# peterWon/D-LIOM

Hardware: AMD Instinct MI355X
Metric: scans/sec (64-beam x 1024 pts -> 10 cm 3D submap) (higher is better)
Workload: dtype f32 transforms + u16 voxels/u64 sums (rtcsm), f64 (ceres); 1 GPU; config2 W-dense: 64x1024 scan, all returns matched (adaptive voxel filters neutralised), RTCSM3D + CeresScanMatcher3D(hi+lo) + insertion(hi+lo); N_hi=65536, N_lo=65536, C=35937, linear_window=1, angular_window=5, rescored_candidates_last=2, box_kernel_variant=0, map_scans=20, grids_inserted_into=2, parallelism=replicas x1

## Files before the change

### d-liom_amd/csrc/internal.h

```cpp
#ifndef DLIOM_CSRC_INTERNAL_H_
#define DLIOM_CSRC_INTERNAL_H_

#include <hip/hip_runtime.h>

#include <chrono>
#include <cstddef>
#include <cstdint>
#include <memory>
#include <string>
#include <vector>

#include "../../include/dliom.h"
#include "pinned_layout.h"

namespace dliom {

void set_last_error(const char* what, hipError_t e, const char* file, int line);

#define DLIOM_HIP_TRY(expr)                                          \
  do {                                                               \
    hipError_t _e = (expr);                                          \
    if (_e != hipSuccess) {                                          \
      ::dliom::set_last_error(#expr, _e, __FILE__, __LINE__);        \
      return DLIOM_ERR_HIP;                                          \
// ... 35 lines not shown
  const uint16_t* dense;
  int dense_stride;
  int dense_bricks;
  int dense_off[3];
};

struct MemoryLedger {
  int64_t grids = 0, leaf_table_bytes = 0, leaf_pool_bytes = 0, mirror_bytes = 0;
  int64_t mirror_budget = 0;
  int64_t outlier_table_bytes = 0;
  int64_t probability_grid_bytes = 0;
  int64_t points_xray_bytes = 0;
  int64_t mirrors_refused = 0;
};

}

struct dliom_ctx {
  std::shared_ptr<dliom::MemoryLedger> ledger = std::make_shared<dliom::MemoryLedger>();
  int device = 0;
  hipStream_t stream = nullptr;
  bool owns_stream = false;
  dliom::DevBuf points;
  dliom::DevBuf cand;
  dliom::DevBuf sums;
  dliom::DevBuf bounds;
  dliom::DevBuf rescore;
  dliom::DevBuf partials;
  dliom::DevBuf misc;
  dliom::DevBuf sort_tmp;
  dliom::DevBuf voxel;
  dliom::DevBuf box_tables;
  dliom::DevBuf box_counters;
  dliom::DevBuf box_extents;
  dliom::DevBuf csm_arrivals;
  dliom::DevBuf box_error;
  dliom::DevBuf deskew_flags;
  unsigned deskew_flag_total = 0;
  unsigned deskew_launch_id = 0;
  int64_t deskew_records_checked = 0, deskew_overflows = 0, deskew_fixed_hits = 0;
  int64_t assemble_recorded = 0, assemble_recomputed = 0, assemble_fixed = 0, assemble_overflows = 0;
  dliom::DevBuf zero_words;
  bool zero_words_ready = false;
  bool box_error_zeroed = false;
  bool force_dense_score = false;
  int tuning[DLIOM_TUNE_COUNT] = {3, 4096, 0};
  bool last_score_used_box = false;
  int last_score_mapping = -1;
  int last_box_refusal = 0;
  int last_box_variant = -1;
  void* pinned = nullptr;
  unsigned* done_word = nullptr;
  unsigned done_seq = 0;
  int64_t voxel_unpacked_reruns = 0;
  int64_t read_backs = 0;
  int64_t poll_fallbacks = 0;
  int64_t host_syncs = 0;
  dliom::DevBuf batch;
  dliom::DevBuf xray_leaves, xray_cells;
  dliom::DevBuf surf, surf_out;
  dliom::DevBuf painter;
  int64_t painter_launches = 0, painter_pairs = 0, painter_texels_uploaded = 0;
  dliom::DevBuf compress, compress_out;
  bool surf_tables_ready = false;
  dliom::DevBuf outlier;
  void* batch_pinned = nullptr;
  size_t batch_pinned_bytes = 0;
  int reserve_batch_pinned(size_t bytes);
  int num_cus = 256;
  unsigned func_attr_set = 0;
  hipStream_t aux_stream = nullptr;
  hipEvent_t aux_fork = nullptr;
  dliom::DevBuf aux_scratch;
  void* aux_pinned = nullptr;
  int aux_histogram_size = 0;
  unsigned aux_seq = 0;
  bool aux_enqueued = false;
  const dliom_cloud* aux_cloud = nullptr;
  float aux_rotation[4] = {1.f, 0.f, 0.f, 0.f};
  bool aux_has_rotation = false;
  bool hist_expect_big = true;
  int hist_poll_us = 150;
  std::chrono::steady_clock::time_point hist_enqueued_at;
  hipStream_t hist_big_stream = nullptr;
  hipEvent_t hist_fork = nullptr, hist_join = nullptr;
  bool profiling = false;
  unsigned profiling_mask = ~0u;
  struct Span {
    hipEvent_t a, b;
    int id;
  };
  std::vector<Span> spans;
  std::vector<hipEvent_t> event_pool;
  double kernel_ms[DLIOM_KERNEL_COUNT] = {};
  int64_t kernel_launches[DLIOM_KERNEL_COUNT] = {};
  dliom_rtcsm_stats last_rtcsm = {};
  void* rtcsm_state = nullptr;
  void (*rtcsm_state_free)(void*) = nullptr;

  int begin_span(int id);
  void end_span(int span);
  int collect_spans();
};

struct dliom_grid {
  dliom_ctx* ctx = nullptr;
  float resolution = 0.f;
  int bits = 1;
  uint32_t* d_table = nullptr;
  uint16_t* d_pool = nullptr;
  int32_t* d_slot_coord = nullptr;
  uint32_t* d_count = nullptr;
  int64_t capacity = 0;
  int64_t used_upper = 1;
  unsigned* h_count_slot = nullptr;
  unsigned insert_seq = 0, applied_seq = 0;
  int64_t upper_at_insert = 0;
  uint16_t* d_dense = nullptr;
  int dense_stride = 0;
  int dense_bricks = 0;
  int dense_off[3] = {0, 0, 0};
  bool dense_windowed = false;
  int64_t dense_rebuilds = 0;
  int ensure_dense();
  int ensure_dense_for(const int centre[3], int radius_cells);
  void drop_dense();
  dliom::GridView view() const;
  std::shared_ptr<dliom::MemoryLedger> ledger;
  int64_t booked_table = 0, booked_pool = 0, booked_mirror = 0;
  int64_t mirror_bytes() const { return d_dense != nullptr ? static_cast<int64_t>(dense_bricks) * dense_bricks * dense_bricks * 128 : 0; }
  void book();
  int ensure_bits(int needed_bits);
  int ensure_capacity(int64_t additional_slots);
  int shrink_to_fit();
  int refresh_count(int64_t* count);
};

struct dliom_cloud {
  dliom_ctx* ctx = nullptr;
  int64_t n = 0;
  int64_t n_padded = 0;
  float* d_x = nullptr;
  float* d_y = nullptr;
  float* d_z = nullptr;
  float* d_xs = nullptr;
  float* d_ys = nullptr;
  float* d_zs = nullptr;
  float max_norm = 0.f;
  float abs_max[3] = {-1.f, -1.f, -1.f};
  bool owned_by_ctx_scratch = false;
  void* base = nullptr;
  size_t base_bytes = 0;
  int device = 0;
  bool morton_ready = false;
  unsigned* d_chunk_order = nullptr;
  unsigned* d_chunk_order_big = nullptr;
};

struct dliom_inserter {
  dliom_ctx* ctx = nullptr;
  int num_free_space_voxels = 0;
  std::vector<uint16_t> hit_table, miss_table;
  uint16_t* d_tables = nullptr;
};


// ... 27 lines not shown
constexpr float kPadCoordinate = 1.0e7f;
int stage_cloud(dliom_ctx* ctx, const float* points_xyz, int64_t n, dliom_cloud* out,
                size_t scratch_offset_bytes = 0);
float cloud_max_norm(const float* points_xyz, int64_t n);
size_t staged_cloud_bytes(int64_t n);
int alloc_device_cloud(dliom_ctx* ctx, int64_t n, dliom_cloud** out, float** x, float** y, float** z);
int finish_device_cloud(dliom_ctx* ctx, dliom_cloud* cloud, float max_norm);
int finish_device_cloud_from(dliom_ctx* ctx, dliom_cloud* cloud, float max_norm, const float* sx, const float* sy, const float* sz);
int ensure_morton(dliom_ctx* ctx, const dliom_cloud* cloud);
struct Soa {
  const float *x, *y, *z, *w;
  int64_t n;
};
int voxel_filter_arrays(dliom_ctx* ctx, const Soa& in, float size, float* ox, float* oy, float* oz, float* ow,
                        int64_t* n_out);
int voxel_filter_arrays_enqueue(dliom_ctx* ctx, const Soa& in, float size, float* ox, float* oy, float* oz, float* ow,
                                const unsigned** d_total, const unsigned** d_unpackable);
int compact_equal_arrays(dliom_ctx* ctx, const Soa& in, const unsigned char* kinds, unsigned char want, float* ox,
                         float* oy, float* oz, int64_t* n_out,
                         const void* also_src = nullptr, unsigned also_words = 0, void* also_dst = nullptr);
int compact_equal_arrays_enqueue(dliom_ctx* ctx, const Soa& in, const unsigned char* kinds, unsigned char want, float* ox,
                                 float* oy, float* oz, const unsigned* n_dev, const unsigned** d_total);
int needed_bits_for_cell_range(int min_index, int max_index);
int project_to_image_on_device(const dliom_grid* grid, const double transform7[7], const uint8_t** image, int32_t* width,
                               int32_t* height, double* ox, double* oy, double* resolution);
int surf_features_on_device(dliom_ctx* ctx, const uint8_t* image, int width, int height, const dliom_surf_options& options,
                            const float** keypoints, const float** descriptors, int* count);
int xray_texture_on_device(const dliom_grid* grid, const double global_submap_pose7[7], const uint8_t** cells, int32_t* width,
                           int32_t* height, double* resolution, double slice_pose7[7]);
int surf_check_options(const dliom_surf_options* options);

constexpr size_t align256(size_t bytes) { return (bytes + 255) & ~static_cast<size_t>(255); }
constexpr unsigned blocks_of(int64_t n, int threads) { return static_cast<unsigned>((n + threads - 1) / threads); }
struct FillJob {
  void* p;
  size_t bytes;
  unsigned value;
};
int fill_multi(dliom_ctx* ctx, const FillJob* jobs, int num_jobs, hipStream_t stream = nullptr);
struct GatherJob {
  const void* src;
  unsigned words;
  unsigned stride = 1;
};
int gather_to_pinned(dliom_ctx* ctx, const GatherJob* jobs, int num_jobs, void* pinned_dst, hipStream_t stream = nullptr,
                     unsigned* done_word = nullptr, unsigned done_seq = 0);
int wait_done(dliom_ctx* ctx, hipStream_t stream, const unsigned* done_word, unsigned done_seq, int max_poll_us = 150);
unsigned next_done_seq(dliom_ctx* ctx);
int gather_and_wait(dliom_ctx* ctx, const GatherJob* jobs, int num_jobs, void* pinned_dst);
int zero_words(dliom_ctx* ctx, unsigned** out);
int device_block_alloc(int device, size_t need, void** p, size_t* bytes);
void device_block_free(int device, void* p, size_t bytes);
struct CompactScratch {
  unsigned *keep, *inclusive, *max_sq;
  int* index;
  void* tmp;
  size_t tmp_bytes;
  void* extra;
};
int carve_compact(dliom_ctx* ctx, int64_t n, CompactScratch* s, size_t extra_bytes = 0, size_t zeroed_extra_bytes = 0);
int empty_cloud(dliom_ctx* ctx, dliom_cloud** out);
int max_of_kept(dliom_ctx* ctx, const float* x, const float* y, const float* z, int64_t n, const CompactScratch& s);
int scan_kept(dliom_ctx* ctx, int64_t n, const CompactScratch& s);
int read_kept(dliom_ctx* ctx, int64_t n, const CompactScratch& s, const GatherJob* more, int64_t* kept, float* max_sq,
              unsigned* more_host);
int emit_kept(dliom_ctx* ctx, const float* x, const float* y, const float* z, int64_t n, const CompactScratch& s, int64_t kept,
              float max_sq, dliom_cloud** out, int32_t* kept_index);
int compact_kept(dliom_ctx* ctx, const dliom_cloud* in, const CompactScratch& s, const unsigned* flag_word, unsigned* flag,
                 dliom_cloud** out, int32_t* kept_index, int64_t capacity, int64_t* num_kept);
int gather_batch_attributes(dliom_ctx* ctx, const int* d_index, int64_t kept, const float* src_intensities, const float* src_colors,
                            float* dst_intensities, float* dst_colors);
int compact_batch(dliom_points_batch* batch, const CompactScratch& s, const unsigned* flag_word, unsigned* flag, int64_t* num_kept);
struct DevicePoints {
  const float4* xyzt;
  const float* intensities;
};
int assemble_from_sensor_points(dliom_ctx* ctx, dliom_trajectory* traj, int64_t cloud_time, const float* points_xyzt, const DevicePoints* device_points,
                                int64_t n, const double sensor_to_tracking[7], dliom_cloud** out, float origin[3], int32_t* kept_index,
                                int64_t capacity, int64_t* num_kept, const float* intensities, AttrBlock* kept_intensities);
int timed_cloud_view(const dliom_timed_cloud* cloud, const dliom_ctx* ctx, int64_t* n, const float4** d_xyzt, const float** d_intensities,
                     float* front_t);
int timed_cloud_origin_index(const dliom_timed_cloud* cloud, bool* has, const float** d_origin_index);
int std_sort_order_enqueue(dliom_ctx* ctx, const float* d_keys, int n, const int** d_order, const int** d_status);
int launch_sequential_sums(dliom_ctx* ctx, int method, const GridView& gv, const dliom_cloud& cloud, const float4* d_rot,
                           int R, const float* d_trans, const unsigned* d_list, const unsigned* d_count, unsigned count,
                           DevBuf* scratch, float* d_ksums);
int sequential_sum_method(int64_t num_points);
int sequential_probability_sums(dliom_ctx* ctx, const dliom_cloud& cloud, const dliom_grid* grid, const float* poses7,
                                int k, float* sums);
struct SequentialSumJob {
  const dliom_cloud* cloud;
  const dliom_grid* grid;
  int first, k;
};
int sequential_probability_sums_enqueue(dliom_ctx* ctx, const SequentialSumJob* jobs, int num_jobs, const float4* d_rot,
                                        const float* d_trans, const unsigned* d_list, float* d_sums);
}

#endif
```

### d-liom_amd/csrc/rtcsm3d.hip

```cpp
#include <algorithm>
#include <cmath>
#include <cstdio>
#include <cstdlib>
#include <cstring>
#include <type_traits>
#include <vector>

#include <dlfcn.h>
#include <rccl/rccl.h>

#include "device_common.h"
#include "host_math.h"
#include "probability_values.h"
#include "rtcsm_candidates.h"
#include "score_box.h"

namespace dliom {

constexpr int kBlock = 256;

template <int PPT, bool WIDE = false>
__global__ __launch_bounds__(kBlock) void rtcsm_score_kernel(
    GridView g, const float* __restrict__ px, const float* __restrict__ py,
    const float* __restrict__ pz, const float4* __restrict__ rot, int R, int r_first, int r_last,
// ... 937 lines not shown
    if (s3 == DLIOM_OK) {
      *pad_processed = 0;
      ctx->last_score_used_box = true;
      ctx->last_score_mapping = 3;
      return DLIOM_OK;
    }
    if (s3 != DLIOM_ERR_CAPACITY) return s3;
    mapping = windowed ? 1 : 2;
  }
  DLIOM_TRY(prep_flush(ctx, &prep));
  ctx->last_score_mapping = mapping;
  int64_t processed = 0;
  if (mapping == 2)
    DLIOM_TRY(launch_score_dense(ctx, cloud, g, c, *d, r_first, r_last, *d_sums, &processed));
  else if (mapping == 1)
    DLIOM_TRY(launch_score_rot(ctx, cloud, g, c, *d, r_first, r_last, *d_sums, &processed));
  else
    DLIOM_TRY(launch_score_point(ctx, cloud, g, c, *d, r_first, r_last, *d_sums, &processed));
  DLIOM_HIP_TRY(hipGetLastError());
  *pad_processed = processed - n;
  return DLIOM_OK;
}

struct LutModel {
  double a, b, delta;
};
static const LutModel& lut_model() {
  static const LutModel m = [] {
    LutModel r;
    r.a = static_cast<double>(kValueToProbabilityScale);
    r.b = static_cast<double>(kValueToProbabilityOffset);
    double d = std::fabs(static_cast<double>(kUnknownProbability) - (r.a * 1.0 + r.b));
    for (int v = 1; v < 32768; ++v) {
      const float f = v * kValueToProbabilityScale + kValueToProbabilityOffset;
      d = std::max(d, std::fabs(static_cast<double>(f) - (r.a * v + r.b)));
    }
    r.delta = d * 1.0000001 + 1e-12;
    return r;
  }();
  return m;
}

static int box_overflowed(dliom_ctx* ctx, unsigned err1, bool* overflow) {
  *overflow = err1 != 0u;
  if (*overflow)
    DLIOM_HIP_TRY(hipMemsetAsync(static_cast<char*>(ctx->box_error.p) + 4, 0, 4, ctx->stream));
  return DLIOM_OK;
}

static int match_begin(dliom_ctx* ctx, const dliom_rtcsm_options* o, const double init7[7],
                       const dliom_cloud& cloud, const dliom_grid* grid, int shard, int num_shards,
                       unsigned* local_best_lo_bits) {
#ifdef DLIOM_EXPERIMENTS
  g_host_prep.start();
#endif
  if (cloud.n <= 0) return DLIOM_ERR_EMPTY_CLOUD;
  if (cloud.n > (1 << 27) || num_shards < 1 || shard < 0 || shard >= num_shards)
    return DLIOM_ERR_INVALID_ARGUMENT;
  RtcsmState* st = state_of(ctx);
  st->active = false;
  st->o = *o;
  st->cloud = cloud;
  st->grid = grid;
  std::memcpy(st->init7, init7, sizeof st->init7);
  st->shard = shard;
  st->num_shards = num_shards;
  st->used_box = false;
  Candidates& c = st->c;
  generate_candidates(*o, grid->resolution, cloud.max_norm, init7, &c);
  DLIOM_PREP_LAP(0);
  const int64_t C = c.w.num_candidates;
  const int R = static_cast<int>(c.w.num_rotations), T = static_cast<int>(c.w.num_translations);
  if (C <= 0 || C > (int64_t{1} << 31)) return DLIOM_ERR_INVALID_ARGUMENT;
  st->r_first = static_cast<int>(static_cast<int64_t>(R) * shard / num_shards);
  st->r_last = static_cast<int>(static_cast<int64_t>(R) * (shard + 1) / num_shards);

  const size_t bytes_f = align256(static_cast<size_t>(C) * 4);
  DLIOM_TRY(ctx->bounds.reserve(3 * bytes_f + 256));
  char* bb = static_cast<char*>(ctx->bounds.p);
  float* d_lo = reinterpret_cast<float*>(bb);
  st->d_hi = reinterpret_cast<float*>(bb + bytes_f);
  st->d_list = reinterpret_cast<unsigned*>(bb + 2 * bytes_f);
  st->d_ctrs = reinterpret_cast<unsigned*>(bb + 3 * bytes_f);
  const FillJob zero_ctrs{st->d_ctrs, 8, 0u};
  if (st->r_last <= st->r_first) DLIOM_TRY(fill_multi(ctx, &zero_ctrs, 1));
  if (st->r_last > st->r_first) {
    int64_t pad_processed = 0;
    DLIOM_TRY(run_score_volume(ctx, cloud, grid, c, st->r_first, st->r_last, &st->d, &st->d_sums,
                               &pad_processed, &zero_ctrs));
    st->used_box = ctx->last_score_used_box;
    const LutModel& lm = lut_model();
    BoundParams bp;
    bp.a = lm.a;
    bp.b = lm.b;
    bp.delta = lm.delta;
    bp.wt = o->translation_delta_cost_weight;
    bp.wr = o->rotation_delta_cost_weight;
    bp.n = static_cast<int>(cloud.n);
    bp.n_pad = static_cast<int>(pad_processed);
    bp.R = R;
    bp.T = T;
    bp.r_first = st->r_first;
    bp.r_last = st->r_last;
    const unsigned cblocks = static_cast<unsigned>((C + 255) / 256);
    const int span = ctx->begin_span(DLIOM_KERNEL_RTCSM_SELECT);
    hipLaunchKernelGGL(rtcsm_bounds_kernel, dim3(cblocks), dim3(256), 0, ctx->stream, st->d_sums,
                       static_cast<long long>(C), st->d.t_norm, st->d.r_angle, bp, d_lo, st->d_hi,
                       st->d_ctrs);
    ctx->end_span(span);
    DLIOM_HIP_TRY(hipGetLastError());
  }
  if (local_best_lo_bits != nullptr) {
    unsigned* h_err = pinned_at<unsigned>(ctx, kPinBoxErrorWord);
    *h_err = 0u;
    DLIOM_HIP_TRY(hipMemcpyAsync(local_best_lo_bits, st->d_ctrs, 4, hipMemcpyDeviceToHost, ctx->stream));
    if (st->used_box)
      DLIOM_HIP_TRY(hipMemcpyAsync(h_err, static_cast<char*>(ctx->box_error.p) + 4, 4, hipMemcpyDeviceToHost, ctx->stream));
    DLIOM_HIP_TRY(hipStreamSynchronize(ctx->stream));
    bool overflow = false;
    DLIOM_TRY(box_overflowed(ctx, *h_err, &overflow));
    if (overflow && !ctx->force_dense_score) {
      ctx->force_dense_score = true;
      const dliom_rtcsm_options o_copy = st->o;
      const int s = match_begin(ctx, &o_copy, init7, cloud, grid, shard, num_shards, local_best_lo_bits);
      ctx->force_dense_score = false;
      return s;
    }
  }
  st->active = true;
  return DLIOM_OK;
}

static int match_finish(dliom_ctx* ctx, const unsigned* global_best_lo_bits, uint64_t* local_best_packed) {
  RtcsmState* st = state_of(ctx);
  if (!st->active) return DLIOM_ERR_INVALID_ARGUMENT;
  const dliom_rtcsm_options* o = &st->o;
  const Candidates& c = st->c;
  const int64_t C = c.w.num_candidates;
  const int R = static_cast<int>(c.w.num_rotations);
  const dliom_cloud& cloud = st->cloud;
  st->best_score = -1.f;
  st->best_c = -1;
  unsigned K = 0;
  if (st->r_last > st->r_first) {
    if (global_best_lo_bits != nullptr) {
      DLIOM_HIP_TRY(hipMemcpyAsync(st->d_ctrs, global_best_lo_bits, 4, hipMemcpyHostToDevice, ctx->stream));
    }
    const unsigned cblocks = static_cast<unsigned>((C + 255) / 256);
    int span = ctx->begin_span(DLIOM_KERNEL_RTCSM_SELECT);
    hipLaunchKernelGGL(rtcsm_select_kernel, dim3(cblocks), dim3(256), 0, ctx->stream, st->d_hi,
                       static_cast<long long>(C), st->d_ctrs, st->d_ctrs + 1, st->d_list);
    ctx->end_span(span);
    DLIOM_HIP_TRY(hipGetLastError());
  }
  constexpr unsigned kSpecK = 8;
  std::vector<unsigned> list;
  std::vector<float> ksums;
  if (st->r_last > st->r_first) {
    static_assert((2 + 2 * kSpecK + 1) * 4 <= kPinMatchReadback.bytes, "the read-back fits its region");
    unsigned* h_ctrs = pinned_at<unsigned>(ctx, kPinMatchReadback);
    unsigned* h_list = h_ctrs + 2;
    float* h_sums = reinterpret_cast<float*>(h_ctrs + 2 + kSpecK);
    auto rescore = [&](unsigned count, const unsigned* d_count, size_t list_offset) -> int {
      DLIOM_TRY(ctx->rescore.reserve(align256(static_cast<size_t>(count) * 4)));
      const int span = ctx->begin_span(DLIOM_KERNEL_RTCSM_RESCORE);
      const int s = launch_sequential_sums(ctx, sequential_sum_method(cloud.n), st->grid->view(), cloud, st->d.rot, R, st->d.trans,
                                           st->d_list + list_offset, d_count, count, &ctx->misc, ctx->rescore.as<float>());
      ctx->end_span(span);
      return s;
    };
    DLIOM_TRY(rescore(kSpecK, st->d_ctrs + 1, 0));
    unsigned* h_err = h_ctrs + 2 + 2 * kSpecK;
    *h_err = 0u;
    const bool want_err = st->used_box && global_best_lo_bits == nullptr;
    const GatherJob back[4] = {{st->d_ctrs, 2}, {st->d_list, kSpecK}, {ctx->rescore.p, kSpecK},
                               {static_cast<char*>(ctx->box_error.p) + 4, 1}};
    DLIOM_TRY(gather_and_wait(ctx, back, want_err ? 4 : 3, h_ctrs));
    {
      bool overflow = false;
      DLIOM_TRY(box_overflowed(ctx, *h_err, &overflow));
      if (overflow && !ctx->force_dense_score) {
        ctx->force_dense_score = true;
        const dliom_rtcsm_options o_copy = st->o;
        const dliom_cloud cloud_copy = st->cloud;
        double init_copy[7];
        std::memcpy(init_copy, st->init7, sizeof init_copy);
        int s = match_begin(ctx, &o_copy, init_copy, cloud_copy, st->grid, st->shard, st->num_shards, nullptr);
        if (s == DLIOM_OK) s = match_finish(ctx, nullptr, local_best_packed);
        ctx->force_dense_score = false;
        return s;
      }
    }
    K = h_ctrs[1];
    const unsigned first = std::min(K, kSpecK);
    list.assign(h_list, h_list + first);
    ksums.assign(h_sums, h_sums + first);
    if (K > kSpecK) {
      const unsigned rest = K - kSpecK;
      DLIOM_TRY(rescore(rest, nullptr, kSpecK));
      list.resize(K);
      ksums.resize(K);
      DLIOM_HIP_TRY(hipMemcpyAsync(list.data() + kSpecK, st->d_list + kSpecK, static_cast<size_t>(rest) * 4,
                                   hipMemcpyDeviceToHost, ctx->stream));
      DLIOM_HIP_TRY(hipMemcpyAsync(ksums.data() + kSpecK, ctx->rescore.p, static_cast<size_t>(rest) * 4,
                                   hipMemcpyDeviceToHost, ctx->stream));
      DLIOM_HIP_TRY(hipStreamSynchronize(ctx->stream));
    }
  }
  if (K > 0) {
    const int n = static_cast<int>(cloud.n);
    for (unsigned k = 0; k < K; ++k) {
      const int64_t cc = list[k];
      const int j = static_cast<int>(cc / R), r = static_cast<int>(cc % R);
      float score = ksums[k];
      score /= static_cast<float>(n);
      const double arg = c.t_norm[j] * o->translation_delta_cost_weight +
                         c.r_angle[r] * o->rotation_delta_cost_weight;
      score *= std::exp(-(arg * (arg * 1.0)));
      if (score > st->best_score || (score == st->best_score && cc < st->best_c)) {
        st->best_score = score;
        st->best_c = cc;
      }
    }
  }
  ctx->last_rtcsm.window = c.w;
  ctx->last_rtcsm.num_points = cloud.n;
  ctx->last_rtcsm.num_rescored = K;
  ctx->last_rtcsm.score_kernel = ctx->last_score_mapping;
  ctx->last_rtcsm.box_kernel_status = ctx->last_box_refusal;
  ctx->last_rtcsm.box_kernel_variant = ctx->last_box_refusal == DLIOM_BOX_RAN ? ctx->last_box_variant : -1;
  ctx->last_rtcsm.best_index = st->best_c;
  if (local_best_packed != nullptr) {
    uint64_t packed = 0;
    if (st->best_c >= 0 && st->best_score > 0.f) {
      uint32_t bits;
      std::memcpy(&bits, &st->best_score, 4);
      packed = (static_cast<uint64_t>(bits) << 32) | (0xFFFFFFFFull - static_cast<uint64_t>(st->best_c));
    }
    *local_best_packed = packed;
  }
  return DLIOM_OK;
}

static int match_decode(dliom_ctx* ctx, uint64_t best_packed, double out7[7], float* out_score) {
  RtcsmState* st = state_of(ctx);
  if (!st->active) return DLIOM_ERR_INVALID_ARGUMENT;
  if (best_packed == 0) return DLIOM_ERR_SCORE_NOT_POSITIVE;
  const Candidates& c = st->c;
  const int R = static_cast<int>(c.w.num_rotations);
  const uint32_t bits = static_cast<uint32_t>(best_packed >> 32);
  const int64_t best_c = static_cast<int64_t>(0xFFFFFFFFull - (best_packed & 0xFFFFFFFFull));
  if (best_c < 0 || best_c >= c.w.num_candidates) return DLIOM_ERR_INVALID_ARGUMENT;
  float score;
  std::memcpy(&score, &bits, 4);
  const int j = static_cast<int>(best_c / R), r = static_cast<int>(best_c % R);
  out7[0] = c.trans[j].x;
  out7[1] = c.trans[j].y;
  out7[2] = c.trans[j].z;
  const QF q = c.rot(static_cast<size_t>(r));
  out7[3] = q.w;
  out7[4] = q.x;
  out7[5] = q.y;
  out7[6] = q.z;
  *out_score = score;
  ctx->last_rtcsm.best_index = best_c;
  return DLIOM_OK;
}

static int match_impl(dliom_ctx* ctx, const dliom_rtcsm_options* o, const double init7[7],
                      const dliom_cloud& cloud, const dliom_grid* grid, double out7[7],
                      float* out_score) {
  DLIOM_TRY(match_begin(ctx, o, init7, cloud, grid, 0, 1, nullptr));
  uint64_t packed = 0;
  DLIOM_TRY(match_finish(ctx, nullptr, &packed));
  return match_decode(ctx, packed, out7, out_score);
}

}

using namespace dliom;

extern "C" {
// ... 290 lines not shown
```

### d-liom_amd/csrc/sequential_sums.hip

```cpp
#include <algorithm>
#include <cstring>
#include <vector>

#include "device_common.h"
#include "probability_values.h"

namespace dliom {

constexpr int kChainTile = 2048;
__global__ __launch_bounds__(256) void rtcsm_rescore_kernel(
    GridView g, const float* __restrict__ px, const float* __restrict__ py,
    const float* __restrict__ pz, int n, const float4* __restrict__ rot, int R,
    const float* __restrict__ trans, const unsigned* __restrict__ list, const unsigned* __restrict__ count,
    float k_scale, float k_offset, float k_unknown, float* __restrict__ sums) {
  __shared__ float4 tile[2][kChainTile / 4];
  if (count != nullptr && blockIdx.x >= *count) return;
  const unsigned c = list[blockIdx.x];
  const int j = static_cast<int>(c / static_cast<unsigned>(R));
  const int r = static_cast<int>(c % static_cast<unsigned>(R));
  const float4 qq = rot[r];
  const Quat4 q{qq.x, qq.y, qq.z, qq.w};
  const float tx = trans[3 * j], ty = trans[3 * j + 1], tz = trans[3 * j + 2];
  const int num_tiles = (n + kChainTile - 1) / kChainTile;
  const int producer = static_cast<int>(threadIdx.x) - 64;
  auto produce = [&](int t) {
    if (producer < 0) return;
    float* dst = reinterpret_cast<float*>(tile[t & 1]);
    for (int k = producer; k < kChainTile; k += 192) {
      const int i = t * kChainTile + k;
      float prob = 0.f;
      if (i < n) {
        float rx, ry, rz;
        rotate_point(q, px[i], py[i], pz[i], rx, ry, rz);
        const unsigned v = grid_value(g, cell_of(rx + tx, g.resolution), cell_of(ry + ty, g.resolution),
                                      cell_of(rz + tz, g.resolution)) & 0x7FFFu;
        prob = v == 0u ? k_unknown : static_cast<float>(static_cast<int>(v)) * k_scale + k_offset;
      }
      dst[k] = prob;
    }
  };
  float s = 0.f;
  produce(0);
  __syncthreads();
  for (int t = 0; t < num_tiles; ++t) {
    if (t + 1 < num_tiles) produce(t + 1);
    if (threadIdx.x == 0) {
      const float4* src = tile[t & 1];
#pragma unroll 8
      for (int k = 0; k < kChainTile / 4; ++k) {
        const float4 v = src[k];
        s += v.x;
        s += v.y;
        s += v.z;
        s += v.w;
      }
    }
    __syncthreads();
  }
  if (threadIdx.x == 0) sums[blockIdx.x] = s;
}

struct ParityFn {
  unsigned s0, s1;
  unsigned p0, p1;
};
__device__ __forceinline__ ParityFn compose(const ParityFn& a, const ParityFn& b) {
  ParityFn r;
  r.s0 = a.s0 + (a.p0 ? b.s1 : b.s0);
  r.p0 = a.p0 ? b.p1 : b.p0;
  r.s1 = a.s1 + (a.p1 ? b.s1 : b.s0);
  r.p1 = a.p1 ? b.p1 : b.p0;
  return r;
}
__device__ __forceinline__ ParityFn shfl_up_fn(const ParityFn& f, int off) {
  ParityFn r;
  r.s0 = __shfl_up(f.s0, off, 64);
  r.s1 = __shfl_up(f.s1, off, 64);
  r.p0 = __shfl_up(f.p0, off, 64);
  r.p1 = __shfl_up(f.p1, off, 64);
  return r;
}

constexpr int kScanThreads = 1024;
constexpr int kSerialPrefix = 256;

__global__ void rtcsm_rescore_values_kernel(GridView g, const float* __restrict__ px,
                                            const float* __restrict__ py, const float* __restrict__ pz,
                                            int n, int n_stride, const float4* __restrict__ rot, int R,
                                            const float* __restrict__ trans, const unsigned* __restrict__ list,
                                            const unsigned* __restrict__ count,
                                            unsigned short* __restrict__ values, float k_scale, float k_offset,
                                            float k_unknown, double* __restrict__ chunk_sums, int num_chunks) {
  if (count != nullptr && blockIdx.y >= *count) return;
  const int i = blockIdx.x * blockDim.x + threadIdx.x;
  unsigned short v = 0;
  if (i < n) {
    const unsigned c = list[blockIdx.y];
    const int j = static_cast<int>(c / static_cast<unsigned>(R));
    const int r = static_cast<int>(c % static_cast<unsigned>(R));
    const float4 qq = rot[r];
    const Quat4 q{qq.x, qq.y, qq.z, qq.w};
    float rx, ry, rz;
    rotate_point(q, px[i], py[i], pz[i], rx, ry, rz);
    v = static_cast<unsigned short>(grid_value(g, cell_of(rx + trans[3 * j], g.resolution),
                                               cell_of(ry + trans[3 * j + 1], g.resolution),
                                               cell_of(rz + trans[3 * j + 2], g.resolution)) & 0x7FFFu);
  }
  if (i < n_stride) values[static_cast<size_t>(blockIdx.y) * n_stride + i] = v;
  if (chunk_sums != nullptr) {
    double p = 0.;
    if (i < n) p = v == 0 ? static_cast<double>(k_unknown)
                          : static_cast<double>(static_cast<float>(static_cast<int>(v)) * k_scale + k_offset);
#pragma unroll
    for (int off = 32; off > 0; off >>= 1) p += __shfl_xor(p, off, 64);
    const int chunk = i >> 6;
    if ((threadIdx.x & 63) == 0 && chunk < num_chunks) chunk_sums[static_cast<size_t>(blockIdx.y) * num_chunks + chunk] = p;
  }
}

__global__ __launch_bounds__(kScanThreads) void rtcsm_rescore_scan_kernel(
    const unsigned short* __restrict__ values, int n, int n_stride, float k_scale, float k_offset,
    float k_unknown, const unsigned* __restrict__ count, float* __restrict__ sums) {
  extern __shared__ unsigned short lds_value[];
  if (count != nullptr && blockIdx.x >= *count) return;
  __shared__ ParityFn wave_total[kScanThreads / 64];
  __shared__ unsigned sh_m, sh_e, sh_i0, sh_cross, sh_m_before, sh_total;
  const int tid = threadIdx.x, lane = tid & 63, wave = tid >> 6;
  {
    const uint4* src = reinterpret_cast<const uint4*>(values + static_cast<size_t>(blockIdx.x) * n_stride);
    uint4* dst = reinterpret_cast<uint4*>(lds_value);
    for (int i = tid; i < n_stride / 8; i += kScanThreads) dst[i] = src[i];
  }
  __syncthreads();
  auto prob = [&](int i) -> float {
    const unsigned v = lds_value[i];
    return v == 0u ? k_unknown : static_cast<float>(static_cast<int>(v)) * k_scale + k_offset;
  };
  auto fixed = [&](int i) -> unsigned {
    const unsigned b = __float_as_uint(prob(i));
    return ((b & 0x7FFFFFu) | 0x800000u) << ((b >> 23) - 123u);
  };
  if (tid == 0) {
// ... 117 lines not shown
  return f;
}
__device__ __forceinline__ unsigned fixed_of_value(unsigned v, float k_scale, float k_offset, float k_unknown) {
  const float p = v == 0u ? k_unknown : static_cast<float>(static_cast<int>(v)) * k_scale + k_offset;
  const unsigned b = __float_as_uint(p);
  return ((b & 0x7FFFFFu) | 0x800000u) << ((b >> 23) - 123u);
}
__device__ __forceinline__ int binade_of(double x) { return max(ilogb(fmax(x, 0.0625)) + 4, 0); }

__global__ __launch_bounds__(256) void rtcsm_rescore_chunk_fns_kernel(
    const unsigned short* __restrict__ values, int n, int n_stride, float k_scale, float k_offset, float k_unknown,
    const unsigned* __restrict__ count, const double* __restrict__ chunk_sums, int num_chunks,
    ChunkFns* __restrict__ fns) {
  if (count != nullptr && blockIdx.y >= *count) return;
  const int lane = threadIdx.x & 63;
  const int c = blockIdx.x * 4 + (threadIdx.x >> 6);
  if (c >= num_chunks) return;
  const double* sums = chunk_sums + static_cast<size_t>(blockIdx.y) * num_chunks;
  double before = 0.;
  for (int k = lane; k < c; k += 64) before += sums[k];
#pragma unroll
  for (int off = 32; off > 0; off >>= 1) before += __shfl_xor(before, off, 64);
  const double after = before + sums[c];
  const int i = c * kChunk + lane;
  const int i_end = min(n, (c + 1) * kChunk);
  const double delta = 1.05 * static_cast<double>(i_end) * 5.9604644775390625e-8 * after + 1e-6;
  const int e_lo = binade_of(before - delta), e_hi = binade_of(after + delta);
  ChunkFns out{0xFFFFFFFFu, 0u, 0u, 0u, 0xFFFFFFFFu, 0u, 0u, 0u};
  if (e_hi - e_lo <= 1) {
    const unsigned a = i < n ? fixed_of_value(values[static_cast<size_t>(blockIdx.y) * n_stride + i], k_scale, k_offset, k_unknown) : 0u;
    const ParityFn id{0u, 0u, 0u, 1u};
    const ParityFn t0 = wave_inclusive_scan(i < n ? element_fn(a, static_cast<unsigned>(e_lo)) : id, lane);
    out.e0 = static_cast<unsigned>(e_lo);
    out.s00 = t0.s0;
    out.s01 = t0.s1;
    out.pp0 = t0.p0 | (t0.p1 << 1);
    if (e_hi != e_lo) {
      const ParityFn t1 = wave_inclusive_scan(i < n ? element_fn(a, static_cast<unsigned>(e_hi)) : id, lane);
      out.e1 = static_cast<unsigned>(e_hi);
      out.s10 = t1.s0;
      out.s11 = t1.s1;
      out.pp1 = t1.p0 | (t1.p1 << 1);
    }
  }
  if (lane == 63) fns[static_cast<size_t>(blockIdx.y) * num_chunks + c] = out;
}

struct PFn2 {
  unsigned a, b;
};
__device__ __forceinline__ PFn2 pfn2_identity() { return PFn2{0u, 0x80000000u}; }
__device__ __forceinline__ PFn2 pack_fn(const ParityFn& f) { return PFn2{f.s0 | (f.p0 << 31), f.s1 | (f.p1 << 31)}; }
__device__ __forceinline__ PFn2 compose2(const PFn2& x, const PFn2& y) {
  PFn2 r;
  r.a = (x.a & 0x7FFFFFFFu) + (static_cast<int>(x.a) < 0 ? y.b : y.a);
  r.b = (x.b & 0x7FFFFFFFu) + (static_cast<int>(x.b) < 0 ? y.b : y.a);
  return r;
}
template <int kCtrl, int kRowMask>
__device__ __forceinline__ PFn2 dpp_fn(const PFn2& f) {
  PFn2 r;
  r.a = static_cast<unsigned>(__builtin_amdgcn_update_dpp(0, static_cast<int>(f.a), kCtrl, kRowMask, 0xf, false));
  r.b = static_cast<unsigned>(__builtin_amdgcn_update_dpp(static_cast<int>(0x80000000u), static_cast<int>(f.b), kCtrl, kRowMask, 0xf, false));
  return r;
}
__device__ __forceinline__ PFn2 wave_inclusive_scan2(PFn2 f) {
  f = compose2(dpp_fn<0x111, 0xf>(f), f);
  f = compose2(dpp_fn<0x112, 0xf>(f), f);
  f = compose2(dpp_fn<0x114, 0xf>(f), f);
  f = compose2(dpp_fn<0x118, 0xf>(f), f);
  f = compose2(dpp_fn<0x142, 0xa>(f), f);
  f = compose2(dpp_fn<0x143, 0xc>(f), f);
  return f;
}
__device__ __forceinline__ PFn2 wave_shift_right1(const PFn2& f) { return dpp_fn<0x138, 0xf>(f); }
__device__ __forceinline__ PFn2 lane_of(const PFn2& f, int l) {
  return PFn2{static_cast<unsigned>(__builtin_amdgcn_readlane(static_cast<int>(f.a), l)),
              static_cast<unsigned>(__builtin_amdgcn_readlane(static_cast<int>(f.b), l))};
}
__device__ __forceinline__ unsigned apply2(const PFn2& f, unsigned parity) { return (parity ? f.b : f.a) & 0x7FFFFFFFu; }

__global__ __launch_bounds__(kScanThreads) void rtcsm_rescore_chunk_scan_kernel(
    const unsigned short* __restrict__ values, int n, int n_stride, float k_scale, float k_offset, float k_unknown,
    const unsigned* __restrict__ count, const ChunkFns* __restrict__ fns, int num_chunks, float* __restrict__ sums) {
  extern __shared__ unsigned short lds_value[];
  if (count != nullptr && blockIdx.x >= *count) return;
  __shared__ PFn2 wave_total[kScanThreads / 64];
  __shared__ unsigned sh_m, sh_e, sh_i0, sh_cross_t, sh_total, sh_mismatch_t, sh_force_serial;
  constexpr int kEarlyChunks = 128;
  __shared__ ChunkFns early_fns[kEarlyChunks];
  const int tid = threadIdx.x, lane = tid & 63, wave = tid >> 6;
  const ChunkFns none{0xFFFFFFFFu, 0u, 0u, 0u, 0xFFFFFFFFu, 0u, 0u, 0u};
  const ChunkFns cf = tid < num_chunks ? fns[static_cast<size_t>(blockIdx.x) * num_chunks + tid] : none;
  if (tid < kEarlyChunks) early_fns[tid] = cf;
  {
    const uint4* src = reinterpret_cast<const uint4*>(values + static_cast<size_t>(blockIdx.x) * n_stride);
    uint4* dst = reinterpret_cast<uint4*>(lds_value);
    for (int i = tid; i < n_stride / 8; i += kScanThreads) dst[i] = src[i];
  }
  __syncthreads();
  auto prob = [&](unsigned v) { return v == 0u ? k_unknown : static_cast<float>(static_cast<int>(v)) * k_scale + k_offset; };
  auto fixed = [&](unsigned i) { return fixed_of_value(lds_value[i], k_scale, k_offset, k_unknown); };
  const int n0 = min(n, kSerialPrefix);
  if (wave == 0) {
    float s = 0.f;
    if (n0 == kSerialPrefix) {
      float pv[kSerialPrefix / 64];
#pragma unroll
      for (int k = 0; k < kSerialPrefix / 64; ++k) pv[k] = prob(lds_value[k * 64 + lane]);
#pragma unroll
      for (int k = 0; k < kSerialPrefix / 64; ++k)
#pragma unroll
        for (int l = 0; l < 64; ++l) s += __int_as_float(__builtin_amdgcn_readlane(__float_as_int(pv[k]), l));
    } else {
      for (int i = 0; i < n0; ++i) s += prob(lds_value[i]);
    }
    const unsigned b0 = __float_as_uint(s);
    unsigned m = (b0 & 0x7FFFFFu) | 0x800000u, e = (b0 >> 23) - 123u, i0 = static_cast<unsigned>(n0);
    const PFn2 idw = pfn2_identity();
    while (i0 < static_cast<unsigned>(n)) {
      const unsigned c_min = max(13421772u >> e, 1u);
      const unsigned window = min(static_cast<unsigned>(n) - i0, ((1u << 24) - m) / c_min + 2u);
      const unsigned c0 = i0 / kChunk;
      const unsigned i_lim = min(static_cast<unsigned>(n), ((i0 + window + kChunk - 1u) / kChunk) * kChunk);
      const unsigned last_chunk = (i_lim - 1u) / kChunk;
      if (last_chunk - c0 >= 64u || last_chunk >= static_cast<unsigned>(kEarlyChunks)) break;
      const unsigned c = c0 + static_cast<unsigned>(lane);
      const unsigned begin = max(i0, c * kChunk), end = min(i_lim, (c + 1u) * kChunk);
      const bool in_window = begin < end;
      PFn2 f = idw;
      bool mismatch = false;
      if (in_window && lane != 0) {
        const ChunkFns cw = early_fns[c];
        if (cw.e0 == e) f = PFn2{cw.s00 | ((cw.pp0 & 1u) << 31), cw.s01 | ((cw.pp0 >> 1) << 31)};
        else if (cw.e1 == e) f = PFn2{cw.s10 | ((cw.pp1 & 1u) << 31), cw.s11 | ((cw.pp1 >> 1) << 31)};
        else mismatch = true;
      }
      {
        const unsigned he = min(i_lim, (c0 + 1u) * kChunk);
        const unsigned i = i0 + static_cast<unsigned>(lane);
        const PFn2 h = wave_inclusive_scan2(i < he ? pack_fn(element_fn(fixed(i), e)) : idw);
        const PFn2 whole = lane_of(h, 63);
        if (lane == 0) f = whole;
      }
      const PFn2 inc = wave_inclusive_scan2(f);
      const PFn2 excl = wave_shift_right1(inc);
      const unsigned p_start = m & 1u;
      const unsigned mt_start = m + apply2(excl, p_start), mt_end = m + apply2(inc, p_start);
      const unsigned long long cross_mask = __ballot(in_window && mt_end >= (1u << 24) && mt_start < (1u << 24));
      const unsigned long long mism_mask = __ballot(mismatch);
      const int cross_l = cross_mask != 0ull ? __ffsll(static_cast<long long>(cross_mask)) - 1 : 64;
      const int mism_l = mism_mask != 0ull ? __ffsll(static_cast<long long>(mism_mask)) - 1 : 64;
      if (mism_l < cross_l || (cross_l == 64 && mism_l != 64)) break;
      if (cross_l == 64) {
        m = static_cast<unsigned>(__builtin_amdgcn_readlane(static_cast<int>(mt_end), 63));
        i0 = i_lim;
        continue;
      }
      const unsigned cb = static_cast<unsigned>(__builtin_amdgcn_readlane(static_cast<int>(begin), cross_l));
      const unsigned ce = static_cast<unsigned>(__builtin_amdgcn_readlane(static_cast<int>(end), cross_l));
      const unsigned ms = static_cast<unsigned>(__builtin_amdgcn_readlane(static_cast<int>(mt_start), cross_l));
      const unsigned i = cb + static_cast<unsigned>(lane);
      const unsigned a_i = i < ce ? fixed(i) : 0u;
      const PFn2 sc = wave_inclusive_scan2(i < ce ? pack_fn(element_fn(a_i, e)) : idw);
      const PFn2 ex = wave_shift_right1(sc);
      const unsigned ps = ms & 1u;
      const unsigned m_before = ms + apply2(ex, ps), m_after = ms + apply2(sc, ps);
      const unsigned long long crossed = __ballot(i < ce && m_after >= (1u << 24));
      if (crossed == 0ull) break;
// ... 23 lines not shown
    const unsigned remaining = static_cast<unsigned>(n) - i0;
    const unsigned window = min(remaining, ((1u << 24) - m) / c_min + 2u);
    const unsigned c0 = i0 / kChunk;
    const unsigned i_lim = min(static_cast<unsigned>(n), ((i0 + window + kChunk - 1u) / kChunk) * kChunk);
    const unsigned c = static_cast<unsigned>(tid);
    const unsigned begin = max(i0, c * kChunk), end = min(i_lim, (c + 1u) * kChunk);
    const bool in_window = begin < end && c >= c0;
    PFn2 f = id;
    bool mismatch = false;
    if (in_window && c != c0) {
      if (cf.e0 == e) f = PFn2{cf.s00 | ((cf.pp0 & 1u) << 31), cf.s01 | ((cf.pp0 >> 1) << 31)};
      else if (cf.e1 == e) f = PFn2{cf.s10 | ((cf.pp1 & 1u) << 31), cf.s11 | ((cf.pp1 >> 1) << 31)};
      else mismatch = true;
    }
    if (mismatch && force_serial) {
      ParityFn g = ParityFn{0u, 0u, 0u, 1u};
      for (unsigned i = begin; i < end; ++i) g = compose(g, element_fn(fixed(i), e));
      f = pack_fn(g);
      mismatch = false;
    }
    if (static_cast<unsigned>(wave) == (c0 >> 6)) {
      const unsigned he = min(i_lim, (c0 + 1u) * kChunk);
      const unsigned i = i0 + static_cast<unsigned>(lane);
      const PFn2 h = wave_inclusive_scan2(i < he ? pack_fn(element_fn(fixed(i), e)) : id);
      const PFn2 whole = lane_of(h, 63);
      if (static_cast<unsigned>(lane) == (c0 & 63u)) f = whole;
    }
    const PFn2 inc = wave_inclusive_scan2(f);
    if (lane == 63) wave_total[wave] = inc;
    if (tid == 0) {
      sh_cross_t = 0xFFFFFFFFu;
      sh_mismatch_t = 0xFFFFFFFFu;
    }
    __syncthreads();
    if (mismatch) atomicMin(&sh_mismatch_t, static_cast<unsigned>(tid));
    PFn2 before = id;
    for (int w = 0; w < wave; ++w) before = compose2(before, wave_total[w]);
    const PFn2 excl = compose2(before, wave_shift_right1(inc));
    const PFn2 incl = compose2(before, inc);
    const unsigned p_start = m & 1u;
    const unsigned mt_start = m + apply2(excl, p_start);
    const unsigned mt_end = m + apply2(incl, p_start);
    if (tid == kScanThreads - 1) sh_total = mt_end - m;
    const bool crosses = in_window && mt_end >= (1u << 24) && mt_start < (1u << 24);
    if (crosses) atomicMin(&sh_cross_t, static_cast<unsigned>(tid));
    __syncthreads();
    const unsigned cross_t = sh_cross_t, mismatch_t = sh_mismatch_t;
    if (mismatch_t < cross_t || (cross_t == 0xFFFFFFFFu && mismatch_t != 0xFFFFFFFFu)) {
      __syncthreads();
      if (tid == 0) sh_force_serial = 1u;
      __syncthreads();
      continue;
    }
    if (cross_t == 0xFFFFFFFFu) {
      if (tid == 0) {
        sh_m = m + sh_total;
        sh_i0 = i_lim;
      }
    } else if (static_cast<unsigned>(wave) == (cross_t >> 6)) {
      const int cl = static_cast<int>(cross_t & 63u);
      const unsigned cb = static_cast<unsigned>(__builtin_amdgcn_readlane(static_cast<int>(begin), cl));
      const unsigned ce = static_cast<unsigned>(__builtin_amdgcn_readlane(static_cast<int>(end), cl));
      const unsigned ms = static_cast<unsigned>(__builtin_amdgcn_readlane(static_cast<int>(mt_start), cl));
      const unsigned i = cb + static_cast<unsigned>(lane);
      const PFn2 sc = wave_inclusive_scan2(i < ce ? pack_fn(element_fn(fixed(i), e)) : id);
      const PFn2 ex = wave_shift_right1(sc);
      const unsigned ps = ms & 1u;
      const unsigned m_before = ms + apply2(ex, ps);
      const unsigned m_after = ms + apply2(sc, ps);
      const unsigned long long crossed = __ballot(i < ce && m_after >= (1u << 24));
      const int first = __ffsll(static_cast<long long>(crossed)) - 1;
      if (lane == first) {
        const unsigned long long X = (static_cast<unsigned long long>(m_before) << e) + fixed(i);
        const unsigned e2 = e + 1u;
        const unsigned long long q2 = X >> e2, f2 = X & ((1ull << e2) - 1ull), h2 = 1ull << e;
        const unsigned long long up = (f2 > h2 || (f2 == h2 && (q2 & 1ull))) ? 1ull : 0ull;
        sh_m = static_cast<unsigned>(q2 + up);
        sh_e = e2;
        sh_i0 = i + 1u;
      }
    }
    __syncthreads();
  }
  if (tid == 0) sums[blockIdx.x] = __uint_as_float(((sh_e + 123u) << 23) | (sh_m & 0x7FFFFFu));
}

constexpr int kRescoreMethod = 2;
constexpr int64_t kRescoreSerialMaxPoints = 1024;

int sequential_sum_method(int64_t num_points) { return num_points <= kRescoreSerialMaxPoints ? 0 : kRescoreMethod; }

struct ScratchLayout {
  size_t sums_at, fns_at, bytes;
};
static ScratchLayout scratch_layout(size_t count, int n) {
  const int n_stride = (n + 7) & ~7, num_chunks = (n + kChunk - 1) / kChunk;
  const size_t values_bytes = align256(count * n_stride * 2), sums_bytes = align256(count * num_chunks * 8);
  return {values_bytes, values_bytes + sums_bytes, values_bytes + sums_bytes + count * num_chunks * sizeof(ChunkFns)};
}

int launch_sequential_sums(dliom_ctx* ctx, int method, const GridView& gv, const dliom_cloud& cloud, const float4* d_rot,
                           int R, const float* d_trans, const unsigned* d_list, const unsigned* d_count, unsigned count,
                           DevBuf* scratch, float* d_ksums) {
  const float k_scale = kValueToProbabilityScale, k_offset = kValueToProbabilityOffset, k_unknown = kUnknownProbability;
  const int n = static_cast<int>(cloud.n);
  const int n_stride = (n + 7) & ~7;
  const size_t scan_lds = static_cast<size_t>(n_stride) * 2;
  if (method == 0 || scan_lds > 128 * 1024 || count > 65535) {
    hipLaunchKernelGGL(rtcsm_rescore_kernel, dim3(count), dim3(256), 0, ctx->stream, gv, cloud.d_x, cloud.d_y, cloud.d_z, n,
                       d_rot, R, d_trans, d_list, d_count, k_scale, k_offset, k_unknown, d_ksums);
    DLIOM_HIP_TRY(hipGetLastError());
    return DLIOM_OK;
  }
  const int num_chunks = (n + kChunk - 1) / kChunk;
  const ScratchLayout at = scratch_layout(count, n);
  DLIOM_TRY(scratch->reserve(at.bytes));
  char* base = static_cast<char*>(scratch->p);
  unsigned short* d_values = reinterpret_cast<unsigned short*>(base);
  double* d_chunk_sums = method == 2 ? reinterpret_cast<double*>(base + at.sums_at) : nullptr;
  ChunkFns* d_fns = reinterpret_cast<ChunkFns*>(base + at.fns_at);
  hipLaunchKernelGGL(rtcsm_rescore_values_kernel, dim3((n_stride + 255) / 256, count), dim3(256), 0, ctx->stream, gv,
                     cloud.d_x, cloud.d_y, cloud.d_z, n, n_stride, d_rot, R, d_trans, d_list, d_count, d_values, k_scale,
                     k_offset, k_unknown, d_chunk_sums, num_chunks);
  if (method == 2) {
    hipLaunchKernelGGL(rtcsm_rescore_chunk_fns_kernel, dim3((num_chunks + 3) / 4, count), dim3(256), 0, ctx->stream, d_values,
                       n, n_stride, k_scale, k_offset, k_unknown, d_count, d_chunk_sums, num_chunks, d_fns);
    hipLaunchKernelGGL(rtcsm_rescore_chunk_scan_kernel, dim3(count), dim3(kScanThreads), scan_lds, ctx->stream, d_values, n,
                       n_stride, k_scale, k_offset, k_unknown, d_count, d_fns, num_chunks, d_ksums);
  } else {
    hipLaunchKernelGGL(rtcsm_rescore_scan_kernel, dim3(count), dim3(kScanThreads), scan_lds, ctx->stream, d_values, n, n_stride,
                       k_scale, k_offset, k_unknown, d_count, d_ksums);
  }
  DLIOM_HIP_TRY(hipGetLastError());
  return DLIOM_OK;
}

int sequential_probability_sums(dliom_ctx* ctx, const dliom_cloud& cloud, const dliom_grid* grid, const float* poses7,
                                int k, float* sums) {
  if (k <= 0 || k > 65535 || cloud.n <= 0) return DLIOM_ERR_INVALID_ARGUMENT;
  const size_t K = static_cast<size_t>(k);
  const size_t rot_bytes = align256(K * 16), trans_bytes = align256(K * 12), list_bytes = align256(K * 4);
  DLIOM_TRY(ctx->bounds.reserve(rot_bytes + trans_bytes + list_bytes));
  std::vector<char> host(rot_bytes + trans_bytes + list_bytes, 0);
  float* hr = reinterpret_cast<float*>(host.data());
  float* ht = reinterpret_cast<float*>(host.data() + rot_bytes);
  unsigned* hl = reinterpret_cast<unsigned*>(host.data() + rot_bytes + trans_bytes);
  for (size_t i = 0; i < K; ++i) {
    const float* p = poses7 + 7 * i;
    hr[4 * i] = p[3];
    hr[4 * i + 1] = p[4];
    hr[4 * i + 2] = p[5];
    hr[4 * i + 3] = p[6];
    ht[3 * i] = p[0];
    ht[3 * i + 1] = p[1];
    ht[3 * i + 2] = p[2];
    hl[i] = static_cast<unsigned>(i * K + i);
  }
  char* base = static_cast<char*>(ctx->bounds.p);
  DLIOM_HIP_TRY(hipMemcpyAsync(base, host.data(), host.size(), hipMemcpyHostToDevice, ctx->stream));
  const float4* d_rot = reinterpret_cast<const float4*>(base);
  const float* d_trans = reinterpret_cast<const float*>(base + rot_bytes);
  const unsigned* d_list = reinterpret_cast<const unsigned*>(base + rot_bytes + trans_bytes);
  DLIOM_TRY(ctx->rescore.reserve(list_bytes));
  float* d_ksums = ctx->rescore.as<float>();
  DLIOM_TRY(launch_sequential_sums(ctx, kRescoreMethod, grid->view(), cloud, d_rot, k, d_trans, d_list, nullptr,
                                   static_cast<unsigned>(k), &ctx->misc, d_ksums));
  if (K <= 1024) {
    const GatherJob job{d_ksums, static_cast<unsigned>(K)};
    static_assert(1024 * 4 <= kPinSequentialSums.bytes, "the sums fit their region");
    float* h = pinned_at<float>(ctx, kPinSequentialSums);
    DLIOM_TRY(gather_and_wait(ctx, &job, 1, h));
    std::memcpy(sums, h, K * 4);
    return DLIOM_OK;
  }
  DLIOM_HIP_TRY(hipMemcpyAsync(sums, d_ksums, K * 4, hipMemcpyDeviceToHost, ctx->stream));
  DLIOM_HIP_TRY(hipStreamSynchronize(ctx->stream));
  ++ctx->host_syncs;
  return DLIOM_OK;
}

int sequential_probability_sums_enqueue(dliom_ctx* ctx, const SequentialSumJob* jobs, int num_jobs, const float4* d_rot,
                                        const float* d_trans, const unsigned* d_list, float* d_sums) {
  size_t most = 0;
  for (int j = 0; j < num_jobs; ++j) {
    if (jobs[j].k <= 0 || jobs[j].k > 65535 || jobs[j].cloud->n <= 0) return DLIOM_ERR_INVALID_ARGUMENT;
    most = std::max(most, scratch_layout(static_cast<size_t>(jobs[j].k), static_cast<int>(jobs[j].cloud->n)).bytes);
  }
  DLIOM_TRY(ctx->misc.reserve(most));
  for (int j = 0; j < num_jobs; ++j) {
    const SequentialSumJob& b = jobs[j];
    DLIOM_TRY(launch_sequential_sums(ctx, kRescoreMethod, b.grid->view(), *b.cloud, d_rot + b.first, b.k, d_trans + 3 * b.first,
                                     d_list + b.first, nullptr, static_cast<unsigned>(b.k), &ctx->misc, d_sums + b.first));
  }
  return DLIOM_OK;
}

}
```

Before: 993.3 scans/s.

## Publish rescore sums directly to pinned memory from the last-arriving block

The rescore kernels now write each candidate's sum, and, in the last block to arrive, the counter pair, candidate list and optional error word, straight into pinned host memory. They then signal a done word that the host polls. This replaces the separate gather copies plus stream synchronisation with an in-kernel system-scope publish and an adaptive poll interval, cutting readback latency on the critical path. It adds an atomic arrival counter (the counter fill grows from 8 to 16 words), system fences, and a dependency on done_word being available. If rescoring ends on method 1 while publishing, the call returns an error.

```diff
diff --git a/d-liom_amd/csrc/internal.h b/d-liom_amd/csrc/internal.h
--- a/d-liom_amd/csrc/internal.h
+++ b/d-liom_amd/csrc/internal.h
@@ -141,6 +141,7 @@
   bool hist_expect_big = true;
   int hist_poll_us = 150;
   std::chrono::steady_clock::time_point hist_enqueued_at;
+  int match_poll_us = 150;
   hipStream_t hist_big_stream = nullptr;
   hipEvent_t hist_fork = nullptr, hist_join = nullptr;
   bool profiling = false;
@@ -334,9 +335,18 @@
                      float* front_t);
 int timed_cloud_origin_index(const dliom_timed_cloud* cloud, bool* has, const float** d_origin_index);
 int std_sort_order_enqueue(dliom_ctx* ctx, const float* d_keys, int n, const int** d_order, const int** d_status);
+constexpr unsigned kSumsPublishHeadWords = 2;
+struct SumsPublish {
+  unsigned* arrivals;
+  unsigned* pinned;
+  const unsigned* head;
+  const unsigned* tail;
+  unsigned* done_word;
+  unsigned done_seq;
+};
 int launch_sequential_sums(dliom_ctx* ctx, int method, const GridView& gv, const dliom_cloud& cloud, const float4* d_rot,
                            int R, const float* d_trans, const unsigned* d_list, const unsigned* d_count, unsigned count,
-                           DevBuf* scratch, float* d_ksums);
+                           DevBuf* scratch, float* d_ksums, const SumsPublish* publish = nullptr);
 int sequential_sum_method(int64_t num_points);
 int sequential_probability_sums(dliom_ctx* ctx, const dliom_cloud& cloud, const dliom_grid* grid, const float* poses7,
                                 int k, float* sums);
diff --git a/d-liom_amd/csrc/rtcsm3d.hip b/d-liom_amd/csrc/rtcsm3d.hip
--- a/d-liom_amd/csrc/rtcsm3d.hip
+++ b/d-liom_amd/csrc/rtcsm3d.hip
@@ -1043,7 +1043,7 @@
   st->d_hi = reinterpret_cast<float*>(bb + bytes_f);
   st->d_list = reinterpret_cast<unsigned*>(bb + 2 * bytes_f);
   st->d_ctrs = reinterpret_cast<unsigned*>(bb + 3 * bytes_f);
-  const FillJob zero_ctrs{st->d_ctrs, 8, 0u};
+  const FillJob zero_ctrs{st->d_ctrs, 16, 0u};
   if (st->r_last <= st->r_first) DLIOM_TRY(fill_multi(ctx, &zero_ctrs, 1));
   if (st->r_last > st->r_first) {
     int64_t pad_processed = 0;
@@ -1122,21 +1122,32 @@
     unsigned* h_ctrs = pinned_at<unsigned>(ctx, kPinMatchReadback);
     unsigned* h_list = h_ctrs + 2;
     float* h_sums = reinterpret_cast<float*>(h_ctrs + 2 + kSpecK);
-    auto rescore = [&](unsigned count, const unsigned* d_count, size_t list_offset) -> int {
+    auto rescore = [&](unsigned count, const unsigned* d_count, size_t list_offset, const SumsPublish* publish) -> int {
       DLIOM_TRY(ctx->rescore.reserve(align256(static_cast<size_t>(count) * 4)));
       const int span = ctx->begin_span(DLIOM_KERNEL_RTCSM_RESCORE);
       const int s = launch_sequential_sums(ctx, sequential_sum_method(cloud.n), st->grid->view(), cloud, st->d.rot, R, st->d.trans,
-                                           st->d_list + list_offset, d_count, count, &ctx->misc, ctx->rescore.as<float>());
+                                           st->d_list + list_offset, d_count, count, &ctx->misc, ctx->rescore.as<float>(), publish);
       ctx->end_span(span);
       return s;
     };
-    DLIOM_TRY(rescore(kSpecK, st->d_ctrs + 1, 0));
+    static_assert(kSumsPublishHeadWords == 2, "the count pair is the block's head");
     unsigned* h_err = h_ctrs + 2 + 2 * kSpecK;
     *h_err = 0u;
     const bool want_err = st->used_box && global_best_lo_bits == nullptr;
-    const GatherJob back[4] = {{st->d_ctrs, 2}, {st->d_list, kSpecK}, {ctx->rescore.p, kSpecK},
-                               {static_cast<char*>(ctx->box_error.p) + 4, 1}};
-    DLIOM_TRY(gather_and_wait(ctx, back, want_err ? 4 : 3, h_ctrs));
+    const unsigned* d_err = reinterpret_cast<const unsigned*>(static_cast<char*>(ctx->box_error.p) + 4);
+    if (ctx->done_word != nullptr) {
+      const SumsPublish publish{st->d_ctrs + 2, h_ctrs, st->d_ctrs, want_err ? d_err : nullptr, ctx->done_word, next_done_seq(ctx)};
+      DLIOM_TRY(rescore(kSpecK, st->d_ctrs + 1, 0, &publish));
+      const auto waiting_since = std::chrono::steady_clock::now();
+      const int waited = wait_done(ctx, ctx->stream, ctx->done_word, publish.done_seq, ctx->match_poll_us);
+      const double took_us = std::chrono::duration<double, std::micro>(std::chrono::steady_clock::now() - waiting_since).count();
+      ctx->match_poll_us = static_cast<int>(std::min(3000.0, std::max(150.0, 2.0 * took_us)));
+      DLIOM_TRY(waited);
+    } else {
+      DLIOM_TRY(rescore(kSpecK, st->d_ctrs + 1, 0, nullptr));
+      const GatherJob back[4] = {{st->d_ctrs, 2}, {st->d_list, kSpecK}, {ctx->rescore.p, kSpecK}, {d_err, 1}};
+      DLIOM_TRY(gather_and_wait(ctx, back, want_err ? 4 : 3, h_ctrs));
+    }
     {
       bool overflow = false;
       DLIOM_TRY(box_overflowed(ctx, *h_err, &overflow));
@@ -1158,7 +1169,7 @@
     ksums.assign(h_sums, h_sums + first);
     if (K > kSpecK) {
       const unsigned rest = K - kSpecK;
-      DLIOM_TRY(rescore(rest, nullptr, kSpecK));
+      DLIOM_TRY(rescore(rest, nullptr, kSpecK, nullptr));
       list.resize(K);
       ksums.resize(K);
       DLIOM_HIP_TRY(hipMemcpyAsync(list.data() + kSpecK, st->d_list + kSpecK, static_cast<size_t>(rest) * 4,
diff --git a/d-liom_amd/csrc/sequential_sums.hip b/d-liom_amd/csrc/sequential_sums.hip
--- a/d-liom_amd/csrc/sequential_sums.hip
+++ b/d-liom_amd/csrc/sequential_sums.hip
@@ -6,15 +6,40 @@
 #include "probability_values.h"
 
 namespace dliom {
+
+__device__ __forceinline__ void publish_sum(const SumsPublish& p, int lane, const unsigned* __restrict__ list, bool has_sum,
+                                            float s) {
+  if (p.done_word == nullptr) return;
+  const unsigned count = gridDim.x;
+  unsigned last = 0u;
+  if (lane == 0) {
+    if (has_sum) reinterpret_cast<float*>(p.pinned)[kSumsPublishHeadWords + count + blockIdx.x] = s;
+    __threadfence_system();
+    last = atomicAdd(p.arrivals, 1u) == count - 1u ? 1u : 0u;
+  }
+  if (__builtin_amdgcn_readfirstlane(static_cast<int>(last)) == 0) return;
+  for (unsigned i = static_cast<unsigned>(lane); i < kSumsPublishHeadWords + count; i += 64u)
+    p.pinned[i] = i < kSumsPublishHeadWords ? p.head[i] : list[i - kSumsPublishHeadWords];
+  if (lane == 0) {
+    if (p.tail != nullptr) p.pinned[kSumsPublishHeadWords + 2u * count] = *p.tail;
+    *p.arrivals = 0u;
+  }
+  __threadfence_system();
+  if (lane == 0) *reinterpret_cast<volatile unsigned*>(p.done_word) = p.done_seq;
+}
+__host__ __device__ inline SumsPublish no_publish() { return SumsPublish{nullptr, nullptr, nullptr, nullptr, nullptr, 0u}; }
 
 constexpr int kChainTile = 2048;
 __global__ __launch_bounds__(256) void rtcsm_rescore_kernel(
     GridView g, const float* __restrict__ px, const float* __restrict__ py,
     const float* __restrict__ pz, int n, const float4* __restrict__ rot, int R,
     const float* __restrict__ trans, const unsigned* __restrict__ list, const unsigned* __restrict__ count,
-    float k_scale, float k_offset, float k_unknown, float* __restrict__ sums) {
+    float k_scale, float k_offset, float k_unknown, float* __restrict__ sums, SumsPublish pub) {
   __shared__ float4 tile[2][kChainTile / 4];
-  if (count != nullptr && blockIdx.x >= *count) return;
+  if (count != nullptr && blockIdx.x >= *count) {
+    if (threadIdx.x < 64) publish_sum(pub, static_cast<int>(threadIdx.x), list, false, 0.f);
+    return;
+  }
   const unsigned c = list[blockIdx.x];
   const int j = static_cast<int>(c / static_cast<unsigned>(R));
   const int r = static_cast<int>(c % static_cast<unsigned>(R));
@@ -58,6 +83,7 @@
     __syncthreads();
   }
   if (threadIdx.x == 0) sums[blockIdx.x] = s;
+  if (threadIdx.x < 64) publish_sum(pub, static_cast<int>(threadIdx.x), list, true, s);
 }
 
 struct ParityFn {
@@ -341,9 +367,13 @@
 
 __global__ __launch_bounds__(kScanThreads) void rtcsm_rescore_chunk_scan_kernel(
     const unsigned short* __restrict__ values, int n, int n_stride, float k_scale, float k_offset, float k_unknown,
-    const unsigned* __restrict__ count, const ChunkFns* __restrict__ fns, int num_chunks, float* __restrict__ sums) {
+    const unsigned* __restrict__ count, const ChunkFns* __restrict__ fns, int num_chunks, float* __restrict__ sums,
+    const unsigned* __restrict__ list, SumsPublish pub) {
   extern __shared__ unsigned short lds_value[];
-  if (count != nullptr && blockIdx.x >= *count) return;
+  if (count != nullptr && blockIdx.x >= *count) {
+    if (threadIdx.x < 64) publish_sum(pub, static_cast<int>(threadIdx.x), list, false, 0.f);
+    return;
+  }
   __shared__ PFn2 wave_total[kScanThreads / 64];
   __shared__ unsigned sh_m, sh_e, sh_i0, sh_cross_t, sh_total, sh_mismatch_t, sh_force_serial;
   constexpr int kEarlyChunks = 128;
@@ -533,7 +563,11 @@
     }
     __syncthreads();
   }
-  if (tid == 0) sums[blockIdx.x] = __uint_as_float(((sh_e + 123u) << 23) | (sh_m & 0x7FFFFFu));
+  if (wave == 0) {
+    const float s = __uint_as_float(((sh_e + 123u) << 23) | (sh_m & 0x7FFFFFu));
+    if (lane == 0) sums[blockIdx.x] = s;
+    publish_sum(pub, lane, list, true, s);
+  }
 }
 
 constexpr int kRescoreMethod = 2;
@@ -552,14 +586,15 @@
 
 int launch_sequential_sums(dliom_ctx* ctx, int method, const GridView& gv, const dliom_cloud& cloud, const float4* d_rot,
                            int R, const float* d_trans, const unsigned* d_list, const unsigned* d_count, unsigned count,
-                           DevBuf* scratch, float* d_ksums) {
+                           DevBuf* scratch, float* d_ksums, const SumsPublish* publish) {
+  const SumsPublish pub = publish != nullptr ? *publish : no_publish();
   const float k_scale = kValueToProbabilityScale, k_offset = kValueToProbabilityOffset, k_unknown = kUnknownProbability;
   const int n = static_cast<int>(cloud.n);
   const int n_stride = (n + 7) & ~7;
   const size_t scan_lds = static_cast<size_t>(n_stride) * 2;
   if (method == 0 || scan_lds > 128 * 1024 || count > 65535) {
     hipLaunchKernelGGL(rtcsm_rescore_kernel, dim3(count), dim3(256), 0, ctx->stream, gv, cloud.d_x, cloud.d_y, cloud.d_z, n,
-                       d_rot, R, d_trans, d_list, d_count, k_scale, k_offset, k_unknown, d_ksums);
+                       d_rot, R, d_trans, d_list, d_count, k_scale, k_offset, k_unknown, d_ksums, pub);
     DLIOM_HIP_TRY(hipGetLastError());
     return DLIOM_OK;
   }
@@ -577,8 +612,9 @@
     hipLaunchKernelGGL(rtcsm_rescore_chunk_fns_kernel, dim3((num_chunks + 3) / 4, count), dim3(256), 0, ctx->stream, d_values,
                        n, n_stride, k_scale, k_offset, k_unknown, d_count, d_chunk_sums, num_chunks, d_fns);
     hipLaunchKernelGGL(rtcsm_rescore_chunk_scan_kernel, dim3(count), dim3(kScanThreads), scan_lds, ctx->stream, d_values, n,
-                       n_stride, k_scale, k_offset, k_unknown, d_count, d_fns, num_chunks, d_ksums);
+                       n_stride, k_scale, k_offset, k_unknown, d_count, d_fns, num_chunks, d_ksums, d_list, pub);
   } else {
+    if (publish != nullptr) return DLIOM_ERR_INVALID_ARGUMENT;
     hipLaunchKernelGGL(rtcsm_rescore_scan_kernel, dim3(count), dim3(kScanThreads), scan_lds, ctx->stream, d_values, n, n_stride,
                        k_scale, k_offset, k_unknown, d_count, d_ksums);
   }
```

Measured after the change: 951.3 scans/s. 0.958x the previous value.
